# facontidavide/cloudini

Hardware: AMD Instinct MI355X
Metric: encode Mpoints/s (stage-1, pre-ZSTD) (higher is better)
Workload: dtype f32->i32 (u8 varint stream); 1 GPU; BASELINE configs[1]: 32 x 1000000-pt XYZI (f32 XYZ + u16 intensity, point_step 16) @1mm, stage-1 encode (pre-LZ4/ZSTD), V5 wire; clouds_per_gpu=32, points_per_cloud=1000000, point_step=16

## Files before the change

### cloudini_amd/csrc/stage1_finish.h

```cpp
#pragma once

namespace cldn {

constexpr uint32_t kFinMaxSegs = 96u + 2u * kMaxAdaptive;
constexpr uint32_t kFinItemUnits = 256u;
constexpr uint32_t kFinMaxItems = 512u;
constexpr uint32_t kFinSpinLimit = 1u << 22;

struct FinishArgs {
  const ChunkDesc* chunks;
  uint32_t n_chunks;
  uint32_t splits;
  const uint32_t* cloud_first_chunk;
  uint32_t n_clouds;
  const uint8_t* slots;
  uint64_t slot_stride;
  const Seg* segs;
  uint32_t segs_per_chunk;
  uint32_t subs;
  unsigned long long* rec;
  unsigned long long* rec2;
  unsigned long long* anchor;
  uint32_t epoch;
  uint32_t* ticket;
// ... 41 lines not shown

__device__ __forceinline__ void fin_layout(FinishLds& L, uint32_t n_segs, uint32_t skip0, uint32_t skip1,
                                           uint32_t dst_mis , uint32_t lane) {
  constexpr uint32_t K = (kFinMaxSegs + 63u) / 64u;
  uint32_t z[K], d[K], cnt[K], ibase[K];
  uint32_t payload = 0u;
#pragma unroll
  for (uint32_t k = 0; k < K; ++k) {
    const uint32_t s = lane + 64u * k;
    z[k] = s < n_segs ? L.seg[s].size : 0u;
    const uint32_t incl = wave_inclusive_scan(z[k]);
    d[k] = payload + incl - z[k];
    payload += (uint32_t)__builtin_amdgcn_readlane((int)incl, 63);
  }
  const uint32_t item_units = max(kFinItemUnits, (payload >> 4) / (kFinMaxItems - kFinMaxSegs - 8u) + 1u);
  uint32_t n_items = 0u;
#pragma unroll
  for (uint32_t k = 0; k < K; ++k) {
    const uint32_t s = lane + 64u * k;
    cnt[k] = 0u;
    if (z[k] != 0u && s != skip0 && s != skip1) {
      const uint32_t head = min(z[k], (16u - ((dst_mis + d[k]) & 15u)) & 15u);
      const uint32_t units = (z[k] - head) >> 4;
      cnt[k] = max(1u, (units + item_units - 1u) / item_units);
    }
    const uint32_t incl = wave_inclusive_scan(cnt[k]);
    ibase[k] = n_items + incl - cnt[k];
    n_items += (uint32_t)__builtin_amdgcn_readlane((int)incl, 63);
  }
#pragma unroll
  for (uint32_t k = 0; k < K; ++k) {
    const uint32_t s = lane + 64u * k;
    if (s < n_segs) L.doff[s] = d[k];
    for (uint32_t j = 0, it = ibase[k]; j < cnt[k] && it < kFinMaxItems; ++j, ++it) {
      L.item_seg[it] = s;
      L.item_u0[it] = j * item_units;
    }
  }
  if (lane == 0u) {
    L.n_items = min(n_items, kFinMaxItems);
    L.item_units = item_units;
    L.payload = payload;
  }
}

__device__ __forceinline__ void fin_copy(const FinishLds& L, const uint8_t* __restrict__ slot, uint8_t* __restrict__ chunk_out,
                                         uint32_t wid, uint32_t n_waves, uint32_t lane) {
  const uint32_t n_items = L.n_items, item_units = L.item_units;
  for (uint32_t it = wid; it < n_items; it += n_waves) {
    const uint32_t sidx = L.item_seg[it], u0 = L.item_u0[it];
    const Seg sg = L.seg[sidx];
    const uint8_t* src = slot + sg.off;
    uint8_t* dst = chunk_out + 4u + L.doff[sidx];
    const uint32_t size = sg.size;
    const uint32_t head = min(size, (uint32_t)((16u - (uint32_t)((uintptr_t)dst & 15u)) & 15u));
    const uint32_t body_units = (size - head) >> 4;
    const uint32_t tail = (size - head) & 15u;
    if (u0 == 0u) {
      if (lane < head) dst[lane] = src[lane];
      if (lane >= 32u && lane < 32u + tail) {
        const uint32_t k = head + body_units * 16u + (lane - 32u);
        dst[k] = src[k];
      }
    }
    const uint32_t sdw = head >> 2, sb = head & 3u;
    const uint4* src4 = reinterpret_cast<const uint4*>(src);
    uint4* dst4 = reinterpret_cast<uint4*>(dst + head);
    const uint32_t u1 = min(body_units, u0 + item_units);
    auto build = [&](const uint4& a, const uint4& b) __attribute__((always_inline)) {
      uint32_t w0, w1, w2, w3, w4;
      switch (sdw) {
        case 0: w0 = a.x; w1 = a.y; w2 = a.z; w3 = a.w; w4 = b.x; break;
        case 1: w0 = a.y; w1 = a.z; w2 = a.w; w3 = b.x; w4 = b.y; break;
        case 2: w0 = a.z; w1 = a.w; w2 = b.x; w3 = b.y; w4 = b.z; break;
        default: w0 = a.w; w1 = b.x; w2 = b.y; w3 = b.z; w4 = b.w; break;
      }
      uint4 o;
      o.x = funnel_bytes(w0, w1, sb);
      o.y = funnel_bytes(w1, w2, sb);
      o.z = funnel_bytes(w2, w3, sb);
      o.w = funnel_bytes(w3, w4, sb);
      return o;
    };
    if (u0 < u1) {
      const uint32_t last = head != 0u ? u1 : u1 - 1u;
      auto shl1 = [&](const uint4& a, const uint4& lane63) __attribute__((always_inline)) {
        uint4 r;
        r.x = (uint32_t)__builtin_amdgcn_update_dpp((int)lane63.x, (int)a.x, 0x130, 0xf, 0xf, false);
        r.y = (uint32_t)__builtin_amdgcn_update_dpp((int)lane63.y, (int)a.y, 0x130, 0xf, 0xf, false);
        r.z = (uint32_t)__builtin_amdgcn_update_dpp((int)lane63.z, (int)a.z, 0x130, 0xf, 0xf, false);
        r.w = (uint32_t)__builtin_amdgcn_update_dpp((int)lane63.w, (int)a.w, 0x130, 0xf, 0xf, false);
        return r;
      };
      auto lane0 = [&](const uint4& a) __attribute__((always_inline)) {
        return make_uint4((uint32_t)__builtin_amdgcn_readfirstlane((int)a.x), (uint32_t)__builtin_amdgcn_readfirstlane((int)a.y),
                          (uint32_t)__builtin_amdgcn_readfirstlane((int)a.z), (uint32_t)__builtin_amdgcn_readfirstlane((int)a.w));
      };
      auto ld = [&](uint32_t j, bool nt) __attribute__((always_inline)) {
        const uint4* q = src4 + min(j, last);
        if (!nt) return *q;
        typedef uint32_t u32x4 __attribute__((ext_vector_type(4)));
        const u32x4 v = __builtin_nontemporal_load(reinterpret_cast<const u32x4*>(q));
        return make_uint4(v.x, v.y, v.z, v.w);
      };
      auto st = [&](uint32_t j, const uint4& v, bool nt) __attribute__((always_inline)) {
        typedef uint32_t u32x4 __attribute__((ext_vector_type(4)));
        u32x4 q;
        q.x = v.x; q.y = v.y; q.z = v.z; q.w = v.w;
        if (nt) __builtin_nontemporal_store(q, reinterpret_cast<u32x4*>(dst4 + j));
        else dst4[j] = v;
      };
      auto rows_loop = [&](auto rows_tag, auto nt_tag) __attribute__((always_inline)) {
        constexpr uint32_t RW = decltype(rows_tag)::value;
        constexpr bool NT = decltype(nt_tag)::value;
        for (uint32_t jb = u0; jb < u1; jb += 64u * RW) {
          const uint32_t j = jb + lane;
          uint4 a[RW + 1];
#pragma unroll
          for (uint32_t r = 0; r < RW; ++r) a[r] = ld(j + 64u * r, NT);
          a[RW] = make_uint4(0u, 0u, 0u, 0u);
          if (lane == 63u && head != 0u) a[RW] = ld(j + 64u * (RW - 1u) + 1u, NT);
#pragma unroll
          for (uint32_t r = 0; r < RW; ++r) {
            const uint4 b = shl1(a[r], r + 1u < RW ? lane0(a[r + 1u]) : a[RW]);
            if (j + 64u * r < u1) st(j + 64u * r, build(a[r], b), NT);
          }
        }
      };
      rows_loop(std::integral_constant<uint32_t, 2>{}, std::true_type{});
    }
  }
}

__global__ __launch_bounds__(256) void k_chunk_sizes(const Seg* __restrict__ segs, uint32_t segs_per_chunk, uint32_t n_chunks,
                                                     uint32_t* __restrict__ chunk_payload, uint32_t* __restrict__ not_contiguous) {
  const uint32_t c = blockIdx.x * 256u + threadIdx.x;
  if (c >= n_chunks) return;
  uint32_t payload = 0u, next = 0xffffffffu;
  bool contiguous = true;
  for (uint32_t s = 0; s < segs_per_chunk; ++s) {
    const Seg sg = segs[(size_t)c * segs_per_chunk + s];
    if (sg.size == 0u) continue;
    if (next != 0xffffffffu && sg.off != next) contiguous = false;
    next = sg.off + sg.size;
    payload += sg.size;
  }
  chunk_payload[c] = payload;
  if (!contiguous) atomicOr(not_contiguous, 1u);
}

template <int T, int FUSE_BPV>
__global__ __launch_bounds__(T, (T == 1024 ? 4 : 8)) __attribute__((amdgpu_num_sgpr(80))) void k_finish(const FinishArgs A) {
  using RawT = typename std::conditional<FUSE_BPV == 4, uint32_t, uint16_t>::type;
  using P = Pal32<RawT>;
  __shared__ FinishLds L;
  extern __shared__ __attribute__((aligned(16))) uint8_t smem[];
  const uint32_t tid = threadIdx.x;
  const uint32_t lane = tid & 63u;
  const uint32_t wave = __builtin_amdgcn_readfirstlane(tid >> 6);

  if (A.test_timeout != 0u && A.use_ticket == 0u) {
    if (tid == 0u && blockIdx.x == 0u) atomicOr(A.status, (uint32_t)ST_FINISH_TIMEOUT);
    return;
  }
  if (tid == 0u) {
    L.ticket = A.use_ticket ? atomicAdd(A.ticket, 1u) : blockIdx.x;
    L.timeout = 0u;
    L.base = 0ull;
  }
  __syncthreads();
  const uint32_t t = L.ticket;
  const uint32_t c = t % A.n_chunks;
  const uint32_t y = t / A.n_chunks;
  const bool leader = (y == 0u);
  const ChunkDesc cd = A.chunks[c];
  const uint32_t n_segs = A.segs_per_chunk;
  if (tid < n_segs) L.seg[tid] = A.segs[(size_t)c * n_segs + tid];

  bool fuse = false, slow = false;
  uint32_t U = 0u;
  const uint32_t n = cd.n_points;
  const RawT* col = nullptr;
  uint16_t* first = nullptr;
  uint32_t s_a = 0xffffffffu, s_b = 0xffffffffu;
  if (FUSE_BPV != 0) {
    fuse = A.modes[cd.cloud * A.n_adaptive + A.fuse_field] == 1u;
    if (fuse) {
      s_a = A.subs + 2u * A.fuse_field;
      s_b = s_a + 1u;
      col = reinterpret_cast<const RawT*>(A.fuse_col) + cd.first_point;
      first = A.fuse_first + cd.first_point;
      if (leader) {
        const P p(smem);
        if (pal32_build<RawT, T>(p, col, n)) {
          U = p.misc[0];
        } else {
          slow = true;
          if (!pal32_slow_first<RawT, T>(p, col, n, first, A.status)) return;
          uint32_t mine = 0u;
          for (uint32_t i = tid; i < n; i += T) mine += first[i] == (uint16_t)i ? 1u : 0u;
          (void)block_exclusive_scan<T>(mine, p.wtot, &U);
          __syncthreads();
        }
        if (tid == 0u) fin_store(A.rec2 + c, ((unsigned long long)A.epoch << 32) | U);
      } else {
        if (tid == 0u) L.pad = fin_wait(A.rec2 + c, A.epoch, L);
        __syncthreads();
        if (L.timeout) {
          if (tid == 0u) atomicOr(A.status, (uint32_t)ST_FINISH_TIMEOUT);
          return;
        }
        U = L.pad;
      }
    }
  }
  __syncthreads();
  if (fuse && tid == 0u) {
    L.seg[s_a].size = 3u + U * (uint32_t)sizeof(RawT);
    L.seg[s_b].size = (palette_bits(U) * n + 7u) >> 3;
  }
  __syncthreads();

  if (tid == 0u) {
    uint32_t payload = 0u;
    for (uint32_t s = 0; s < n_segs; ++s) payload += L.seg[s].size;
    L.payload = payload;
    if (leader) fin_store(A.rec + c, ((unsigned long long)A.epoch << 32) | (payload + 4u));
  }
  {
    unsigned long long part = 0ull;
    const uint32_t blk = c >> 10;
    {
      constexpr uint32_t PER = 1024u / T;
      unsigned long long x[PER];
#pragma unroll
      for (uint32_t k = 0; k < PER; ++k) {
        const uint32_t j = (blk << 10) + tid + k * T;
        x[k] = j < c ? fin_load(A.rec + j) : ((unsigned long long)A.epoch << 32);
      }
      if (FUSE_BPV != 0 && fuse && leader && !slow) (void)pal32_rank<RawT, T>(P(smem), nullptr);
#pragma unroll
      for (uint32_t k = 0; k < PER; ++k) {
        const uint32_t j = (blk << 10) + tid + k * T;
        part += (uint32_t)(x[k] >> 32) == A.epoch ? (uint32_t)x[k] : fin_wait(A.rec + j, A.epoch, L);
      }
    }
    if (blk != 0u && tid == T - 1) {
      for (uint32_t spins = 0;; ++spins) {
        const unsigned long long x = fin_load(A.anchor + (blk - 1u));
        if (x != 0ull) {
          part += x - 1ull;
          break;
        }
        if (spins >= kFinSpinLimit || ((spins & 255u) == 255u && *(volatile uint32_t*)&L.timeout != 0u)) {
          L.timeout = 1u;
          break;
        }
        __builtin_amdgcn_s_sleep(2);
      }
    }
    uint32_t lo = (uint32_t)part, hi = (uint32_t)(part >> 32);
#pragma unroll
    for (int d = 32; d >= 1; d >>= 1) {
      const uint32_t olo = (uint32_t)__shfl_down((int)lo, d), ohi = (uint32_t)__shfl_down((int)hi, d);
      const unsigned long long sum = ((((unsigned long long)hi) << 32) | lo) + ((((unsigned long long)ohi) << 32) | olo);
      lo = (uint32_t)sum;
      hi = (uint32_t)(sum >> 32);
    }
    if (lane == 0u && (lo | hi)) atomicAdd(&L.base, (((unsigned long long)hi) << 32) | lo);
  }
  __syncthreads();
  if (L.timeout) {
    if (tid == 0u) atomicOr(A.status, (uint32_t)ST_FINISH_TIMEOUT);
    return;
  }
  const unsigned long long dst0 = L.base;
  if (wave == 0u) fin_layout(L, n_segs, s_a, s_b, (uint32_t)(((uintptr_t)A.out + dst0 + 4ull) & 15ull), lane);
  __syncthreads();
  const uint32_t payload = L.payload;
  if (dst0 + 4ull + payload > A.out_capacity) {
    if (tid == 0u && leader) atomicOr(A.status, (uint32_t)ST_OUT_OVERFLOW);
    return;
  }
  uint8_t* chunk_out = A.out + dst0;
  if (leader) {
    if (tid < 4u) chunk_out[tid] = (uint8_t)(payload >> (8u * tid));
    if (tid == 0u) {
      A.chunk_payload[c] = payload;
      A.chunk_dst[c] = dst0;
      if ((c & 1023u) == 1023u) fin_store(A.anchor + (c >> 10), dst0 + 4ull + payload + 1ull);
    }
    if (tid == 64u) {
      for (uint32_t k = cd.cloud + 1u; k-- > 0u && A.cloud_first_chunk[k] == c;) A.stream_offsets[k] = dst0;
      if (c + 1u == A.n_chunks)
        for (uint32_t k = A.n_clouds + 1u; k-- > 0u && A.cloud_first_chunk[k] == A.n_chunks;) A.stream_offsets[k] = dst0 + 4ull + payload;
    }
  }

  const uint8_t* slot = A.slots + (size_t)c * A.slot_stride;
  const bool leader_copies = !(fuse && A.splits >= 3u);
  const uint32_t wid = leader_copies ? y * (T / 64) + wave : (y - 1u) * (T / 64) + wave;
  const uint32_t n_waves = (leader_copies ? A.splits : A.splits - 1u) * (T / 64);
  const bool copies = leader_copies || !leader;
  const bool section_first = !fuse || !leader || (c & 1u) == 0u;
  if (!section_first && copies) fin_copy(L, slot, chunk_out, wid, n_waves, lane);
  if (FUSE_BPV != 0 && fuse && leader) {
    const P p(smem);
    uint8_t* sec = chunk_out + 4u + L.doff[s_a];
    uint8_t* idx = chunk_out + 4u + L.doff[s_b];
    if (!slow) {
      pal32_values<RawT, T>(p, sec + 3u);
      pal32_pack_chunk<RawT, T>(p, col, n, palette_bits(U), idx);
    } else {
      (void)pal32_slow_rank<RawT, T>(p, col, n, first, sec + 3u);
      pal32_slow_pack<RawT, T>(p, n, palette_bits(U), first, idx);
    }
    if (tid == 0u) {
      sec[0] = 1u;
      sec[1] = (uint8_t)(U & 0xffu);
      sec[2] = (uint8_t)((U >> 8) & 0xffu);
    }
  }
  if (section_first && copies) fin_copy(L, slot, chunk_out, wid, n_waves, lane);
}

}
```

### cloudini_amd/csrc/stage1_sections.h

```cpp
#pragma once

namespace cldn {

constexpr uint32_t kPalSeed = 2048u;

constexpr int kS2Threads = 1024;
constexpr uint32_t kS2PalSlots = 4096;
constexpr uint32_t kS2PalCapacity = 3072;
constexpr uint32_t kInf = 0xffffffffu;
constexpr uint32_t kProbeSlots = 8192;
constexpr uint32_t kProbeLds = kProbeSlots * 8u + 16u + 256u;

struct Pal2 {
  unsigned long long* keys;
  uint32_t* first;
  uint16_t* rank;
  uint32_t* misc;
  uint32_t* wtot;
};
constexpr uint32_t kS2PalLds = kS2PalSlots * 8u + (kS2PalSlots + 4u) * 4u + (kS2PalSlots + 8u) * 2u + 16u + 256u;

__device__ __forceinline__ Pal2 pal2_carve(uint8_t* lds) {
  Pal2 p;
  uint32_t o = 0;
// ... 167 lines not shown
    for (uint32_t w = threadIdx.x; w < 2048u; w += T) bm[w] = 0u;
    __syncthreads();
#pragma unroll
    for (uint32_t j = 0; j < VPT; ++j)
      if (j < cnt) atomicOr(&bm[(uint32_t)v[j] >> 5], 1u << ((uint32_t)v[j] & 31u));
    __syncthreads();
    uint32_t pc = 0u;
    for (uint32_t w = threadIdx.x; w < 2048u; w += T) pc += (uint32_t)__builtin_popcount(bm[w]);
    U = block_sum<T>(pc, wtot);
  } else {
    using Key = typename std::conditional<sizeof(RawT) == 8, unsigned long long, uint32_t>::type;
    constexpr Key kFreeKey = ~(Key)0;
    Key* keys = reinterpret_cast<Key*>(smem);
    uint32_t* cnt_l = wtot + 40;
    for (uint32_t sidx = threadIdx.x; sidx < slots; sidx += T) keys[sidx] = kFreeKey;
    if (threadIdx.x < 2u) cnt_l[threadIdx.x] = 0u;
    __syncthreads();
#pragma unroll
    for (uint32_t j = 0; j < VPT; ++j) {
      if (j < cnt) {
        const Key key = (Key)v[j];
        if (key == kFreeKey) {
          cnt_l[1] = 1u;
        } else {
          const uint32_t h32 = sizeof(RawT) == 8 ? hash_u64((uint64_t)key) * 0x9e3779b1u : (uint32_t)key * 0x9e3779b1u;
          uint32_t slot = (uint32_t)(((uint64_t)h32 * slots) >> 32);
          for (;;) {
            Key k = keys[slot];
            if (k == kFreeKey) {
              k = atomicCAS(&keys[slot], kFreeKey, key);
              if (k == kFreeKey) {
                atomicAdd(&cnt_l[0], 1u);
                break;
              }
            }
            if (k == key) break;
            slot = slot + 1u == slots ? 0u : slot + 1u;
          }
        }
      }
    }
    __syncthreads();
    U = cnt_l[0] + cnt_l[1];
    __syncthreads();
  }
  const uint32_t pal_size = 3u + U * (uint32_t)sizeof(RawT) + ((palette_bits(U) * n + 7u) >> 3);

  uint32_t mode = 0u, best = delta_size;
  if (pal_size < best) { best = pal_size; mode = 1u; }
  if (rle_size < best) { best = rle_size; mode = 2u; }
  if (drle_size < best) { mode = 3u; }
  return (uint8_t)mode;
}

template <typename RawT>
__device__ __forceinline__ uint8_t probe_mode(const RawT* col, uint32_t n, uint32_t type, uint8_t* smem) {
  uint32_t* wtot = reinterpret_cast<uint32_t*>(smem + kProbeSlots * 8u + 16u);
  return probe_mode_t<RawT, kS2Threads>([&](uint32_t i) { return col[i]; }, n, type, smem, kProbeSlots, wtot);
}

__global__ __launch_bounds__(kS2Threads) void k_probe_fast(const DevPlan plan, const ChunkDesc* __restrict__ chunks,
                                                           const uint32_t* __restrict__ cloud_first_chunk,
                                                           const ColumnPtrs cols, uint8_t* __restrict__ modes) {
  extern __shared__ __attribute__((aligned(16))) uint8_t smem[];
  const uint32_t cloud = blockIdx.x, a = blockIdx.y;
  uint8_t* mode_out = modes + cloud * plan.n_adaptive + a;
  const uint32_t fc = cloud_first_chunk[cloud];
  if (fc == cloud_first_chunk[cloud + 1u]) {
    if (threadIdx.x == 0) *mode_out = 0u;
    return;
  }
  const ChunkDesc cd = chunks[fc];
  const uint32_t n = cd.n_points > kProbePoints ? kProbePoints : cd.n_points;
  const uint32_t bpv = plan.adaptive[a].bpv, type = plan.adaptive[a].type;
  const uint8_t* col = cols.p[a] + (size_t)cd.first_point * bpv;
  uint8_t mode;
  if (bpv == 2u) mode = probe_mode<uint16_t>(reinterpret_cast<const uint16_t*>(col), n, type, smem);
  else if (bpv == 4u) mode = probe_mode<uint32_t>(reinterpret_cast<const uint32_t*>(col), n, type, smem);
  else mode = probe_mode<uint64_t>(reinterpret_cast<const uint64_t*>(col), n, type, smem);
  if (threadIdx.x == 0) *mode_out = mode;
}

template <typename RawT>
__global__ __launch_bounds__(kS2Threads) void k_section_palette(const DevPlan plan, const SectionFields fl,
                                                                const ChunkDesc* __restrict__ chunks,
                                                                const ColumnPtrs cols, const uint8_t* __restrict__ modes,
                                                                uint8_t* __restrict__ slots, uint64_t slot_stride,
                                                                uint64_t reg_stride, Seg* __restrict__ segs,
                                                                uint32_t segs_per_chunk, uint32_t subs,
                                                                uint8_t* __restrict__ handled_flags, uint32_t ) {
  constexpr int T = kS2Threads;
  constexpr int NW = T / 64;
  constexpr uint32_t ROUND = T * 8u;
  extern __shared__ __attribute__((aligned(16))) uint8_t smem[];
  const uint32_t c = blockIdx.x;
  const uint32_t a = fl.a[blockIdx.y];
  const ChunkDesc cd = chunks[c];
  if (modes[cd.cloud * plan.n_adaptive + a] != 1u) return;
  const uint32_t n = cd.n_points;
  const RawT* col = reinterpret_cast<const RawT*>(cols.p[a]) + cd.first_point;
  const uint32_t sec_off = (uint32_t)reg_stride + a * kSectionStride;
  uint8_t* dst = slots + (size_t)c * slot_stride + sec_off;
  const Pal2 p = pal2_carve(smem);
  const uint32_t tid = threadIdx.x;
  const uint32_t lane = tid & 63u;
  const uint32_t wave = __builtin_amdgcn_readfirstlane(tid >> 6);
  const uint32_t rounds = (n + ROUND - 1u) / ROUND;

  for (uint32_t s = tid; s < kS2PalSlots; s += T) p.keys[s] = ~0ull;
  for (uint32_t s = tid; s <= kS2PalSlots; s += T) p.first[s] = kInf;
  if (tid < 4u) p.misc[tid] = 0u;
  __syncthreads();

  for (uint32_t r = 0; r < rounds; ++r) {
    const uint32_t i0 = r * ROUND + tid * 8u;
    if (i0 < n) {
      RawT v[8];
      load8<RawT>(col, i0, n, v);
#pragma unroll
      for (int j = 0; j < 8; ++j) {
        if (i0 + (uint32_t)j < n) pal2_insert<RawT>(p, v[j], i0 + (uint32_t)j);
      }
    }
  }
  __syncthreads();
  if (p.misc[1] != 0u || p.misc[0] > kS2PalCapacity) return;

  uint32_t fmask = 0u;
  uint32_t incl[4], cnt[4];
#pragma unroll
  for (uint32_t r = 0; r < 4u; ++r) {
    uint32_t m = 0u;
    const uint32_t i0 = r * ROUND + tid * 8u;
    if (r < rounds && i0 < n) {
      RawT v[8];
      load8<RawT>(col, i0, n, v);
#pragma unroll
      for (int j = 0; j < 8; ++j) {
        if (i0 + (uint32_t)j < n && p.first[pal2_find<RawT>(p, v[j])] == i0 + (uint32_t)j) m |= 1u << j;
      }
    }
    fmask |= m << (8u * r);
    cnt[r] = (uint32_t)__builtin_popcount(m);
    incl[r] = wave_inclusive_scan(cnt[r]);
    if (lane == 63u) p.wtot[r * NW + wave] = incl[r];
  }
  __syncthreads();
  const uint32_t wincl = wave_inclusive_scan(p.wtot[lane]);
  const uint32_t U = (uint32_t)__builtin_amdgcn_readlane((int)wincl, 63);
#pragma unroll
  for (uint32_t r = 0; r < 4u; ++r) {
    const int f = (int)(r * NW + wave);
    const uint32_t rowbase = (f == 0) ? 0u : (uint32_t)__builtin_amdgcn_readlane((int)wincl, f - 1);
    const uint32_t m = (fmask >> (8u * r)) & 0xffu;
    if (m) {
      uint32_t rk = rowbase + incl[r] - cnt[r];
      const uint32_t i0 = r * ROUND + tid * 8u;
      RawT v[8];
      load8<RawT>(col, i0, n, v);
#pragma unroll
      for (int j = 0; j < 8; ++j) {
        if (m & (1u << j)) {
          p.rank[pal2_find<RawT>(p, v[j])] = (uint16_t)rk;
          const unsigned long long val = (unsigned long long)v[j];
          uint8_t* out = dst + 3u + (size_t)rk * sizeof(RawT);
#pragma unroll
          for (uint32_t k = 0; k < sizeof(RawT); ++k) out[k] = (uint8_t)(val >> (8u * k));
          ++rk;
        }
      }
    }
  }
  if (tid == 0) {
    dst[0] = 1u;
    dst[1] = (uint8_t)(U & 0xffu);
    dst[2] = (uint8_t)((U >> 8) & 0xffu);
  }
  __syncthreads();

  const uint32_t bits = palette_bits(U);
  if (bits != 0u && tid * 32u < n) {
    uint32_t* idx_out = reinterpret_cast<uint32_t*>(dst + kPaletteIndexOffset) + (size_t)tid * bits;
    uint64_t scratch = 0u;
    uint32_t held = 0u, w = 0u;
    for (uint32_t g = 0; g < 4u; ++g) {
      const uint32_t i0 = tid * 32u + g * 8u;
      if (i0 >= n) break;
      RawT v[8];
      load8<RawT>(col, i0, n, v);
#pragma unroll
      for (int j = 0; j < 8; ++j) {
        if (i0 + (uint32_t)j < n) {
          scratch |= ((uint64_t)p.rank[pal2_find<RawT>(p, v[j])]) << held;
          held += bits;
          if (held >= 32u) {
            idx_out[w++] = (uint32_t)scratch;
            scratch >>= 32;
            held -= 32u;
          }
        }
      }
    }
    if (held > 0u) idx_out[w] = (uint32_t)scratch;
  }
  if (tid == 0) {
    Seg s;
    s.off = sec_off;
    s.size = 3u + U * (uint32_t)sizeof(RawT);
    segs[(size_t)c * segs_per_chunk + subs + 2u * a] = s;
    s.off = sec_off + kPaletteIndexOffset;
    s.size = (bits * n + 7u) >> 3;
    segs[(size_t)c * segs_per_chunk + subs + 1u + 2u * a] = s;
    handled_flags[(size_t)c * plan.n_adaptive + a] = 1u;
  }
}

template <typename RawT>
struct Grp8 {
  uint32_t dw[2 * sizeof(RawT)];
  __device__ __forceinline__ uint32_t get(int j) const {
    return sizeof(RawT) == 2 ? ((dw[j >> 1] >> ((j & 1) * 16)) & 0xffffu) : dw[j];
  }
  __device__ __forceinline__ uint32_t get_dyn(uint32_t j) const {
    const uint32_t di = sizeof(RawT) == 2 ? (j >> 1) : j;
    uint32_t x = 0u;
#pragma unroll
    for (uint32_t k = 0; k < 2 * sizeof(RawT); ++k) {
      uint32_t a = dw[k];
      asm volatile("" : "+v"(a));
      x = di == k ? a : x;
    }
    return sizeof(RawT) == 2 ? ((x >> ((j & 1u) * 16u)) & 0xffffu) : x;
  }
};
template <typename RawT>
__device__ __forceinline__ Grp8<RawT> grp8_load(const RawT* col, uint32_t i0) {
  Grp8<RawT> g;
  __builtin_memcpy(g.dw, col + i0, 8u * sizeof(RawT));
  return g;
}

template <typename RawT>
struct Pal32 {
  using Word = typename std::conditional<sizeof(RawT) == 2, uint32_t, unsigned long long>::type;
  static constexpr uint32_t kShift = sizeof(RawT) == 2 ? 16u : 32u;
  static constexpr Word kFree = ~(Word)0;
  static constexpr uint32_t kLds = kS2PalSlots * (uint32_t)sizeof(Word) + 2u * kS2Threads * 4u + 16u + 256u;
  Word* tab;
  uint32_t* bitmap;
  uint32_t* prefix;
  uint32_t* misc;
  uint32_t* wtot;
  __device__ __forceinline__ explicit Pal32(uint8_t* lds) {
    uint32_t o = 0;
    tab = reinterpret_cast<Word*>(lds + o);
    o += kS2PalSlots * (uint32_t)sizeof(Word);
    bitmap = reinterpret_cast<uint32_t*>(lds + o);
    o += kS2Threads * 4u;
    prefix = reinterpret_cast<uint32_t*>(lds + o);
    o += kS2Threads * 4u;
    misc = reinterpret_cast<uint32_t*>(lds + o);
    o += 16u;
    wtot = reinterpret_cast<uint32_t*>(lds + o);
  }
  static __device__ __forceinline__ uint32_t home(uint32_t v) { return (v * 0x9e3779b1u) >> 20; }
  static __device__ __forceinline__ uint32_t key_of(Word w) { return (uint32_t)(w >> kShift); }
  static __device__ __forceinline__ uint32_t low_of(Word w) { return (uint32_t)w & 0xffffu; }

  __device__ __forceinline__ void insert(uint32_t v, uint32_t index, Word w) const {
    const Word mine = ((Word)v << kShift) | index;
    uint32_t slot = home(v);
    uint32_t probes = 0u;
    for (;;) {
      if (misc[0] > kS2PalCapacity) return;
      if (w == kFree) {
        w = atomicCAS(&tab[slot], kFree, mine);
        if (w == kFree) {
          atomicAdd(&misc[0], 1u);
          return;
        }
      }
      if (key_of(w) == v) {
        if (low_of(w) > index) atomicMin(&tab[slot], mine);
        return;
      }
      slot = (slot + 1u) & (kS2PalSlots - 1u);
      if (++probes > kS2PalSlots) {
        misc[1] = 1u;
        return;
      }
      w = tab[slot];
    }
  }
  __device__ __forceinline__ uint32_t find_rank(uint32_t v, Word w) const {
    uint32_t slot = home(v);
    while (w == kFree || key_of(w) != v) {
      slot = (slot + 1u) & (kS2PalSlots - 1u);
      w = tab[slot];
    }
    return low_of(w);
  }
};

template <typename RawT, uint32_t BITS, bool AHEAD = false>
__device__ __forceinline__ void pal32_pack(const Pal32<RawT>& p, const RawT* col, uint32_t i0, uint32_t n, uint32_t cnt,
                                           uint8_t* out) {
  using P = Pal32<RawT>;
  uint32_t w[BITS];
#pragma unroll
  for (uint32_t k = 0; k < BITS; ++k) w[k] = 0u;
  Grp8<RawT> grp[AHEAD ? 4 : 1];
  if constexpr (AHEAD) {
#pragma unroll
    for (int g = 0; g < 4; ++g) grp[g] = grp8_load<RawT>(col, i0 + 8u * g < n ? i0 + 8u * g : i0);
  }
#pragma unroll
  for (int g = 0; g < 4; ++g) {
    uint32_t v[8];
    if constexpr (AHEAD) {
#pragma unroll
      for (int j = 0; j < 8; ++j) v[j] = grp[g].get(j);
    } else {
      RawT rv[8];
#pragma unroll
      for (int j = 0; j < 8; ++j) rv[j] = (RawT)0;
      if (i0 + 8u * g < n) load8<RawT>(col, i0 + 8u * g, n, rv);
#pragma unroll
      for (int j = 0; j < 8; ++j) v[j] = (uint32_t)rv[j];
    }
    typename P::Word tw[8];
#pragma unroll
    for (int j = 0; j < 8; ++j) tw[j] = p.tab[P::home(v[j])];
#pragma unroll
    for (int j = 0; j < 8; ++j) {
      const uint32_t e = (uint32_t)(8 * g + j);
      uint32_t x = 0u;
      if (e < cnt) {
        const bool hit = tw[j] != P::kFree && P::key_of(tw[j]) == v[j];
        x = hit ? P::low_of(tw[j]) : p.find_rank(v[j], tw[j]);
      }
      const uint32_t bit = e * BITS;
      w[bit >> 5] |= x << (bit & 31u);
      if ((bit & 31u) + BITS > 32u) w[(bit >> 5) + 1u] |= x >> (32u - (bit & 31u));
    }
  }
  const uint32_t n_bytes = (cnt * BITS + 7u) >> 3;
  const uint32_t n_dw = n_bytes >> 2;
  if (n_dw == BITS && BITS % 4u == 0u) {
#pragma unroll
    for (uint32_t k = 0; k < BITS; k += 4u) {
      const uint4 q = make_uint4(w[k], w[k + 1u], w[k + 2u], w[k + 3u]);
      __builtin_memcpy(out + 4u * k, &q, 16);
    }
  } else {
#pragma unroll
    for (uint32_t k = 0; k < BITS; ++k) {
      if (k < n_dw) __builtin_memcpy(out + 4u * k, &w[k], 4);
      else if (k == n_dw) {
        for (uint32_t b = 0; b < (n_bytes & 3u); ++b) out[4u * k + b] = (uint8_t)(w[k] >> (8u * b));
      }
    }
  }
}


template <typename RawT, int T>
__device__ __forceinline__ bool pal32_build(const Pal32<RawT>& p, const RawT* col, uint32_t n) {
  using P = Pal32<RawT>;
  using Word = typename P::Word;
  constexpr uint32_t WPT = kS2Threads / T;
  const uint32_t tid = threadIdx.x;
  uint32_t seedv[kPalSeed / T];
#pragma unroll
  for (uint32_t r = 0; r < kPalSeed / T; ++r) seedv[r] = (uint32_t)col[min(r * T + tid, n - 1u)];
  for (uint32_t s = tid; s < kS2PalSlots; s += T) p.tab[s] = P::kFree;
#pragma unroll
  for (uint32_t w = 0; w < WPT; ++w) p.bitmap[w * T + tid] = 0u;
  if (tid < 4u) p.misc[tid] = 0u;
  __syncthreads();
#pragma unroll
  for (uint32_t r = 0; r < kPalSeed / T; ++r) {
    const uint32_t i = r * T + tid;
    if (i < n) p.insert(seedv[r], i, p.tab[P::home(seedv[r])]);
  }
  __syncthreads();
  constexpr uint32_t STEPS = 4096u / T;
  constexpr uint32_t GB = sizeof(RawT) == 2 ? (STEPS < 8u ? STEPS : 8u) : 4u;
#pragma unroll
  for (uint32_t b = 0; b < STEPS; b += GB) {
    Grp8<RawT> g[GB];
#pragma unroll
    for (uint32_t k = 0; k < GB; ++k) {
      const uint32_t i0 = ((b + k) * T + tid) * 8u;
      g[k] = grp8_load<RawT>(col, i0 < n ? i0 : 0u);
    }
#pragma unroll
    for (uint32_t k = 0; k < GB; ++k) {
      const uint32_t i0 = ((b + k) * T + tid) * 8u;
      if (i0 >= n || i0 + 8u <= kPalSeed) continue;
      Word w[8];
#pragma unroll
      for (int j = 0; j < 8; ++j) w[j] = p.tab[P::home(g[k].get(j))];
      uint32_t todo = 0u;
#pragma unroll
      for (int j = 0; j < 8; ++j) {
        const uint32_t idx = i0 + (uint32_t)j;
        const bool settled = w[j] != P::kFree && P::key_of(w[j]) == g[k].get(j) && P::low_of(w[j]) <= idx;
        todo |= (idx < n && !settled) ? (1u << j) : 0u;
      }
      while (todo != 0u) {
        const uint32_t j = (uint32_t)__builtin_ctz(todo);
        todo &= todo - 1u;
        const uint32_t v = g[k].get_dyn(j);
        p.insert(v, i0 + j, p.tab[P::home(v)]);
      }
    }
  }
  __syncthreads();
  return p.misc[1] == 0u && p.misc[0] <= kS2PalCapacity;
}

template <typename RawT, int T>
__device__ __forceinline__ uint32_t pal32_rank(const Pal32<RawT>& p, uint8_t* vals_out) {
  using P = Pal32<RawT>;
  using Word = typename P::Word;
  constexpr uint32_t WPT = kS2Threads / T;
  const uint32_t tid = threadIdx.x;
#pragma unroll
  for (uint32_t q = 0; q < kS2PalSlots / T; ++q) {
    const Word w = p.tab[q * T + tid];
    if (w != P::kFree) atomicOr(&p.bitmap[P::low_of(w) >> 5], 1u << (P::low_of(w) & 31u));
  }
  __syncthreads();
  uint32_t U;
  {
    uint32_t pc[WPT], mine = 0u;
#pragma unroll
    for (uint32_t w = 0; w < WPT; ++w) {
      pc[w] = (uint32_t)__builtin_popcount(p.bitmap[WPT * tid + w]);
      mine += pc[w];
    }
    uint32_t run = block_exclusive_scan<T>(mine, p.wtot, &U);
#pragma unroll
    for (uint32_t w = 0; w < WPT; ++w) {
      p.prefix[WPT * tid + w] = run;
      run += pc[w];
    }
  }
  __syncthreads();
#pragma unroll
  for (uint32_t q = 0; q < kS2PalSlots / T; ++q) {
    const Word w = p.tab[q * T + tid];
    if (w != P::kFree) {
      const uint32_t f = P::low_of(w);
      const uint32_t rk = p.prefix[f >> 5] + (uint32_t)__builtin_popcount(p.bitmap[f >> 5] & ((1u << (f & 31u)) - 1u));
      p.tab[q * T + tid] = (w & ~(Word)0xffffu) | rk;
      if (vals_out != nullptr) {
        const uint32_t val = P::key_of(w);
        uint8_t* out = vals_out + (size_t)rk * sizeof(RawT);
#pragma unroll
        for (uint32_t b = 0; b < sizeof(RawT); ++b) out[b] = (uint8_t)(val >> (8u * b));
      }
    }
  }
  __syncthreads();
  return U;
}

template <typename RawT, int T>
__device__ __forceinline__ void pal32_values(const Pal32<RawT>& p, uint8_t* vals_out) {
  using P = Pal32<RawT>;
  using Word = typename P::Word;
  const uint32_t tid = threadIdx.x;
#pragma unroll
  for (uint32_t q = 0; q < kS2PalSlots / T; ++q) {
    const Word w = p.tab[q * T + tid];
    if (w != P::kFree) {
      const uint32_t val = P::key_of(w);
      uint8_t* out = vals_out + (size_t)P::low_of(w) * sizeof(RawT);
#pragma unroll
      for (uint32_t b = 0; b < sizeof(RawT); ++b) out[b] = (uint8_t)(val >> (8u * b));
    }
  }
}

template <typename RawT, int T>
__device__ __forceinline__ void pal32_pack_chunk(const Pal32<RawT>& p, const RawT* col, uint32_t n, uint32_t bits,
                                                 uint8_t* idx_out) {
  constexpr uint32_t WPT = kS2Threads / T;
  const uint32_t tid = threadIdx.x;
  for (uint32_t g = 0; g < WPT; ++g) {
    const uint32_t grp = g * T + tid;
    const uint32_t i0 = grp * 32u;
    const uint32_t cnt = i0 < n ? min(32u, n - i0) : 0u;
    if (bits != 0u && cnt != 0u) {
      uint8_t* o = idx_out + (size_t)grp * bits * 4u;
      switch (bits) {
        case 1: pal32_pack<RawT, 1, T == 1024>(p, col, i0, n, cnt, o); break;
        case 2: pal32_pack<RawT, 2, T == 1024>(p, col, i0, n, cnt, o); break;
        case 3: pal32_pack<RawT, 3, T == 1024>(p, col, i0, n, cnt, o); break;
        case 4: pal32_pack<RawT, 4, T == 1024>(p, col, i0, n, cnt, o); break;
        case 5: pal32_pack<RawT, 5, T == 1024>(p, col, i0, n, cnt, o); break;
        case 6: pal32_pack<RawT, 6, T == 1024>(p, col, i0, n, cnt, o); break;
        case 7: pal32_pack<RawT, 7, T == 1024>(p, col, i0, n, cnt, o); break;
        case 8: pal32_pack<RawT, 8, T == 1024>(p, col, i0, n, cnt, o); break;
        case 9: pal32_pack<RawT, 9, T == 1024>(p, col, i0, n, cnt, o); break;
        case 10: pal32_pack<RawT, 10, T == 1024>(p, col, i0, n, cnt, o); break;
        case 11: pal32_pack<RawT, 11, T == 1024>(p, col, i0, n, cnt, o); break;
        default: pal32_pack<RawT, 12, T == 1024>(p, col, i0, n, cnt, o); break;
      }
    }
  }
}

constexpr uint32_t kPalSlowMaxParts = 4096;

template <typename RawT>
__device__ __forceinline__ uint32_t pal32_part(uint32_t v, uint32_t parts) {
  if (sizeof(RawT) == 2) return (v * parts) >> 16;
  uint32_t h = v * 0x85ebca6bu;
  h ^= h >> 15;
  h *= 0xc2b2ae35u;
  return (uint32_t)(((uint64_t)h * parts) >> 32);
}

template <typename RawT, int T>
__device__ __forceinline__ bool pal32_slow_first(const Pal32<RawT> p, const RawT* col, uint32_t n, uint16_t* first, uint32_t* status) {
  using P = Pal32<RawT>;
  const uint32_t tid = threadIdx.x;
  uint32_t parts = 32u;
  for (;;) {
    bool ok = true;
    for (uint32_t part = 0; part < parts && ok; ++part) {
      __syncthreads();
      for (uint32_t s = tid; s < kS2PalSlots; s += T) p.tab[s] = P::kFree;
      if (tid < 4u) p.misc[tid] = 0u;
      __syncthreads();
      for (uint32_t i = tid; i < n; i += T) {
        const uint32_t v = (uint32_t)col[i];
        if (pal32_part<RawT>(v, parts) == part) p.insert(v, i, p.tab[P::home(v)]);
      }
      __syncthreads();
      ok = p.misc[1] == 0u && p.misc[0] <= kS2PalCapacity;
      if (!ok) break;
      for (uint32_t i = tid; i < n; i += T) {
        const uint32_t v = (uint32_t)col[i];
        if (pal32_part<RawT>(v, parts) == part) {
          uint32_t slot = P::home(v);
          typename P::Word w = p.tab[slot];
          while (w == P::kFree || P::key_of(w) != v) {
            slot = (slot + 1u) & (kS2PalSlots - 1u);
            w = p.tab[slot];
          }
          first[i] = (uint16_t)P::low_of(w);
        }
      }
    }
    if (ok) break;
    if (sizeof(RawT) == 2 || parts >= kPalSlowMaxParts) {
      if (tid == 0) atomicOr(status, (uint32_t)ST_PALETTE_FULL);
      return false;
    }
    parts *= 4u;
  }
  __threadfence_block();
  __syncthreads();
  return true;
}

template <typename RawT, int T>
__device__ __forceinline__ uint32_t pal32_slow_rank(const Pal32<RawT> p, const RawT* col, uint32_t n, const uint16_t* first,
                                    uint8_t* vals_out) {
  constexpr uint32_t WPT = kS2Threads / T;
  const uint32_t tid = threadIdx.x;
  uint32_t U;
  uint32_t pc[WPT], bm[WPT], mine = 0u;
#pragma unroll
  for (uint32_t w = 0; w < WPT; ++w) {
    const uint32_t word = WPT * tid + w;
    uint32_t m = 0u;
    for (uint32_t b = 0; b < 32u; ++b) {
      const uint32_t i = word * 32u + b;
      if (i < n && first[i] == (uint16_t)i) m |= 1u << b;
    }
    bm[w] = m;
    p.bitmap[word] = m;
    pc[w] = (uint32_t)__builtin_popcount(m);
    mine += pc[w];
  }
  uint32_t run = block_exclusive_scan<T>(mine, p.wtot, &U);
#pragma unroll
  for (uint32_t w = 0; w < WPT; ++w) {
    const uint32_t word = WPT * tid + w;
    p.prefix[word] = run;
    uint32_t m = bm[w];
    uint32_t rk = run;
    while (m) {
      const uint32_t b = (uint32_t)__builtin_ctz(m);
      m &= m - 1u;
      const uint64_t val = (uint64_t)col[word * 32u + b];
      uint8_t* out = vals_out + (size_t)rk * sizeof(RawT);
#pragma unroll
      for (uint32_t k = 0; k < sizeof(RawT); ++k) out[k] = (uint8_t)(val >> (8u * k));
      ++rk;
    }
    run += pc[w];
  }
  __syncthreads();
  return U;
}

template <typename RawT, int T>
__device__ __forceinline__ void pal32_slow_pack(const Pal32<RawT> p, uint32_t n, uint32_t bits, const uint16_t* first, uint8_t* idx_out) {
  constexpr uint32_t WPT = kS2Threads / T;
  const uint32_t tid = threadIdx.x;
  if (bits == 0u) return;
  for (uint32_t g = 0; g < WPT; ++g) {
    const uint32_t grp = g * T + tid;
    const uint32_t i0 = grp * 32u;
    if (i0 >= n) continue;
    const uint32_t cnt = min(32u, n - i0);
    uint8_t* o = idx_out + (size_t)grp * bits * 4u;
    uint64_t scratch = 0u;
    uint32_t held = 0u, w = 0u;
    for (uint32_t j = 0; j < cnt; ++j) {
      const uint32_t f = first[i0 + j];
      const uint32_t rk = p.prefix[f >> 5] + (uint32_t)__builtin_popcount(p.bitmap[f >> 5] & ((1u << (f & 31u)) - 1u));
      scratch |= ((uint64_t)rk) << held;
      held += bits;
      if (held >= 32u) {
        const uint32_t d = (uint32_t)scratch;
        __builtin_memcpy(o + 4u * w, &d, 4);
        ++w;
        scratch >>= 32;
        held -= 32u;
      }
    }
    for (uint32_t b = 0; b < ((held + 7u) >> 3); ++b) o[4u * w + b] = (uint8_t)(scratch >> (8u * b));
  }
}

template <typename RawT, int T = kS2Threads>
__global__ __launch_bounds__(T, (T == 512 ? 8 : 4)) __attribute__((amdgpu_num_sgpr(80))) void k_section_palette32(
    const DevPlan plan, const SectionFields fl, const ChunkDesc* __restrict__ chunks, const ColumnPtrs cols,
    const uint8_t* __restrict__ modes, uint8_t* __restrict__ slots, uint64_t slot_stride, uint64_t reg_stride,
    Seg* __restrict__ segs, uint32_t segs_per_chunk, uint32_t subs, uint8_t* __restrict__ handled_flags, uint32_t append,
    const ColumnPtrs first_cols, uint32_t* __restrict__ status) {
  static_assert(sizeof(RawT) == 2 || sizeof(RawT) == 4, "16- or 32-bit keys");
  static_assert(kS2Threads * 32u == 32768u && (T == kS2Threads || 2 * T == kS2Threads), "bitmap words per thread: 1 or 2");
  using P = Pal32<RawT>;
  extern __shared__ __attribute__((aligned(16))) uint8_t smem[];
  const uint32_t c = blockIdx.x;
  const uint32_t a = fl.a[blockIdx.y];
  const ChunkDesc cd = chunks[c];
  if (modes[cd.cloud * plan.n_adaptive + a] != 1u) return;
  const uint32_t n = cd.n_points;
  const RawT* col = reinterpret_cast<const RawT*>(cols.p[a]) + cd.first_point;
  const uint32_t sec_off = append ? segs[(size_t)c * segs_per_chunk].size : (uint32_t)reg_stride + a * kSectionStride;
  uint8_t* dst = slots + (size_t)c * slot_stride + sec_off;
  const P p(smem);
  const uint32_t tid = threadIdx.x;

  uint32_t U;
  if (pal32_build<RawT, T>(p, col, n)) {
    U = p.misc[0];
    (void)pal32_rank<RawT, T>(p, dst + 3u);
    pal32_pack_chunk<RawT, T>(p, col, n, palette_bits(U), dst + 3u + U * (uint32_t)sizeof(RawT));
  } else {
    uint16_t* first = reinterpret_cast<uint16_t*>(first_cols.p[a]) + cd.first_point;
    if (!pal32_slow_first<RawT, T>(p, col, n, first, status)) return;
    uint32_t mine = 0u;
    for (uint32_t i = tid; i < n; i += T) mine += first[i] == (uint16_t)i ? 1u : 0u;
    (void)block_exclusive_scan<T>(mine, p.wtot, &U);
    __syncthreads();
    (void)pal32_slow_rank<RawT, T>(p, col, n, first, dst + 3u);
    pal32_slow_pack<RawT, T>(p, n, palette_bits(U), first, dst + 3u + U * (uint32_t)sizeof(RawT));
  }
  if (tid == 0) {
    dst[0] = 1u;
    dst[1] = (uint8_t)(U & 0xffu);
    dst[2] = (uint8_t)((U >> 8) & 0xffu);
    Seg s;
    s.off = sec_off;
    s.size = 3u + U * (uint32_t)sizeof(RawT) + ((palette_bits(U) * n + 7u) >> 3);
    segs[(size_t)c * segs_per_chunk + subs + 2u * a] = s;
    s.size = 0u;
    segs[(size_t)c * segs_per_chunk + subs + 1u + 2u * a] = s;
    handled_flags[(size_t)c * plan.n_adaptive + a] = 1u;
  }
}

constexpr uint32_t kD32Ring = 65536;
constexpr uint32_t kD32Lds = kD32Ring + 256u;

template <typename RawT>
__device__ __forceinline__ void section_delta32_body(const DevPlan& plan, uint32_t c, uint32_t a, const ChunkDesc& cd, const ColumnPtrs& cols,
                                                     uint8_t* __restrict__ slots, uint64_t slot_stride, uint64_t reg_stride,
                                                     Seg* __restrict__ segs, uint32_t segs_per_chunk, uint32_t subs,
                                                     uint8_t* __restrict__ handled_flags, uint32_t append, uint8_t* smem) {
  static_assert(sizeof(RawT) == 2 || sizeof(RawT) == 4, "differences of at most 33 bits");
  constexpr int T = kS2Threads;
  uint32_t* ring = reinterpret_cast<uint32_t*>(smem);
  uint32_t* wtot = reinterpret_cast<uint32_t*>(smem + kD32Ring);
  const uint32_t n = cd.n_points;
  const uint32_t type = plan.adaptive[a].type;
  const RawT* col = reinterpret_cast<const RawT*>(cols.p[a]) + cd.first_point;
  const uint32_t sec_off = append ? segs[(size_t)c * segs_per_chunk].size : (uint32_t)reg_stride + a * kSectionStride;
  uint8_t* dst = slots + (size_t)c * slot_stride + sec_off;
  const uint32_t tid = threadIdx.x;
  Grp8<RawT> pre[4];
  RawT pre_prev[4];
#pragma unroll
  for (uint32_t q = 0; q < 4u; ++q) {
    const uint32_t i0 = q * (T * 8u) + threadIdx.x * 8u;
    pre[q] = grp8_load<RawT>(col, i0 < n ? i0 : 0u);
    pre_prev[q] = col[(i0 > 0u && i0 < n) ? i0 - 1u : 0u];
  }
  for (uint32_t i = tid; i < kD32Ring / 16u; i += T) reinterpret_cast<uint4*>(ring)[i] = make_uint4(0u, 0u, 0u, 0u);
  __syncthreads();

  uint32_t R = 1u, F = 0u;
#pragma unroll
  for (uint32_t q = 0; q < 4u; ++q) {
    const uint32_t i0 = q * (T * 8u) + tid * 8u;
    if (q * (T * 8u) >= n) break;
    RawT v[8];
#pragma unroll
    for (int j = 0; j < 8; ++j) v[j] = (RawT)pre[q].get(j);
    int64_t prev = (i0 > 0u && i0 < n) ? int_field_as_i64((uint64_t)pre_prev[q], type) : 0;
    uint32_t w0[8], w1[8], lens = 0u, total = 0u;
#pragma unroll
    for (int j = 0; j < 8; ++j) {
      const int64_t cur = int_field_as_i64((uint64_t)v[j], type);
      const int64_t d = (int64_t)((uint64_t)cur - (uint64_t)prev);
      prev = cur;
      const uint64_t u = (((uint64_t)d << 1) ^ (uint64_t)(d >> 63)) + 1ull;
      const uint32_t bl = (u >> 32) ? (64u - (uint32_t)__builtin_clzll(u)) : (32u - (uint32_t)__builtin_clz((uint32_t)u));
      const uint32_t l = (i0 + (uint32_t)j < n) ? groups7(bl) : 0u;
      w0[j] = spread28((uint32_t)u & 0x0fffffffu) | cont_mask(l ? l - 1u : 0u);
      w1[j] = (uint32_t)(u >> 28);
      lens |= l << (4 * j);
      total += l;
    }
    uint32_t tile_total;
    uint32_t off = R + block_exclusive_scan<T>(total, wtot, &tile_total);
#pragma unroll
    for (int j = 0; j < 8; ++j) {
      const uint32_t l = (lens >> (4 * j)) & 0xfu;
      if (l) ring_put5<kD32Ring, false>(ring, off, w0[j], w1[j], l, 0u);
      off += l;
    }
    const uint32_t r_end = R + tile_total;
    const bool last = (q + 1u) * (T * 8u) >= n;
    const uint32_t target = last ? ((r_end + 15u) & ~15u) : (r_end & ~15u);
    __syncthreads();
    ring_flush_n<T, kD32Ring>(ring, dst, F, target);
    F = target;
    R = r_end;
    __syncthreads();
  }
  if (tid == 0) {
    Seg sg;
    sg.off = sec_off;
    sg.size = R;
    segs[(size_t)c * segs_per_chunk + subs + 2u * a] = sg;
    sg.off = sec_off;
    sg.size = 0u;
    segs[(size_t)c * segs_per_chunk + subs + 1u + 2u * a] = sg;
    handled_flags[(size_t)c * plan.n_adaptive + a] = 1u;
  }
}

template <typename RawT>
__device__ __forceinline__ void section_runs_body(const DevPlan& plan, uint32_t c, uint32_t a, const ChunkDesc& cd, uint32_t mode,
                                                  const ColumnPtrs& cols, uint8_t* __restrict__ slots, uint64_t slot_stride,
                                                  uint64_t reg_stride, Seg* __restrict__ segs, uint32_t segs_per_chunk, uint32_t subs,
                                                  uint8_t* __restrict__ handled_flags, uint32_t append, uint8_t* smem) {
  static_assert(sizeof(RawT) == 2 || sizeof(RawT) == 4, "differences of at most 33 bits");
  constexpr int T = kS2Threads;
  uint32_t* wtot = reinterpret_cast<uint32_t*>(smem);
  const bool delta = (mode == 3u);
  const uint32_t n = cd.n_points;
  const uint32_t type = plan.adaptive[a].type;
  const RawT* col = reinterpret_cast<const RawT*>(cols.p[a]) + cd.first_point;
  const uint32_t sec_off = append ? segs[(size_t)c * segs_per_chunk].size : (uint32_t)reg_stride + a * kSectionStride;
  uint8_t* dst = slots + (size_t)c * slot_stride + sec_off;
  const uint32_t tid = threadIdx.x;
  const uint32_t i0 = tid * 32u;
  const uint32_t cnt = i0 < n ? min(32u, n - i0) : 0u;
  auto as64 = [&](RawT r) { return int_field_as_i64((uint64_t)r, type); };

  uint64_t key[32];
  uint64_t key_before = 0u;
  {
    RawT v[32];
    Grp8<RawT> g8[4];
#pragma unroll
    for (uint32_t g = 0; g < 4u; ++g) g8[g] = grp8_load<RawT>(col, i0 + 8u * g < n ? i0 + 8u * g : 0u);
    const RawT pm1r = col[(cnt && i0 >= 1u) ? i0 - 1u : 0u];
    const RawT pm2r = col[(cnt && i0 >= 2u) ? i0 - 2u : 0u];
#pragma unroll
    for (int g = 0; g < 4; ++g)
#pragma unroll
      for (int j = 0; j < 8; ++j) v[8 * g + j] = (i0 + (uint32_t)(8 * g + j) < n) ? (RawT)g8[g].get(j) : (RawT)0;
    const RawT pm1 = (cnt && i0 >= 1u) ? pm1r : (RawT)0;
    const RawT pm2 = (cnt && i0 >= 2u) ? pm2r : (RawT)0;
    if (delta) {
      int64_t prev = i0 >= 1u ? as64(pm1) : 0;
      key_before = (uint64_t)prev - (uint64_t)(i0 >= 2u ? as64(pm2) : 0);
#pragma unroll
      for (int j = 0; j < 32; ++j) {
        const int64_t cur = as64(v[j]);
        key[j] = (uint64_t)cur - (uint64_t)prev;
        prev = cur;
// ... 89 lines not shown
```

Baseline: 133,800 Mpoints/s.

## Repack palette indices per 8-value group with batched loads and deferred misses

The palette index packer now gives each thread one 8-value group per step instead of 32 values, so consecutive threads write adjacent small outputs. Loads for several groups are issued up front, separated from the compute by a scheduling barrier. Hash-table misses are collected into a bitmask and resolved afterwards, and base pointers are forced uniform with readfirstlane. The copy ordering in the finish step is also simplified to always run after palette emission. This trades more loop iterations and some register pressure for better coalescing and latency hiding.

```diff
diff --git a/cloudini_amd/csrc/stage1_finish.h b/cloudini_amd/csrc/stage1_finish.h
--- a/cloudini_amd/csrc/stage1_finish.h
+++ b/cloudini_amd/csrc/stage1_finish.h
@@ -367,8 +367,6 @@
   const uint32_t wid = leader_copies ? y * (T / 64) + wave : (y - 1u) * (T / 64) + wave;
   const uint32_t n_waves = (leader_copies ? A.splits : A.splits - 1u) * (T / 64);
   const bool copies = leader_copies || !leader;
-  const bool section_first = !fuse || !leader || (c & 1u) == 0u;
-  if (!section_first && copies) fin_copy(L, slot, chunk_out, wid, n_waves, lane);
   if (FUSE_BPV != 0 && fuse && leader) {
     const P p(smem);
     uint8_t* sec = chunk_out + 4u + L.doff[s_a];
@@ -386,7 +384,7 @@
       sec[2] = (uint8_t)((U >> 8) & 0xffu);
     }
   }
-  if (section_first && copies) fin_copy(L, slot, chunk_out, wid, n_waves, lane);
-}
-
-}
+  if (copies) fin_copy(L, slot, chunk_out, wid, n_waves, lane);
+}
+
+}
diff --git a/cloudini_amd/csrc/stage1_sections.h b/cloudini_amd/csrc/stage1_sections.h
--- a/cloudini_amd/csrc/stage1_sections.h
+++ b/cloudini_amd/csrc/stage1_sections.h
@@ -493,64 +493,55 @@
   }
 };
 
-template <typename RawT, uint32_t BITS, bool AHEAD = false>
-__device__ __forceinline__ void pal32_pack(const Pal32<RawT>& p, const RawT* col, uint32_t i0, uint32_t n, uint32_t cnt,
-                                           uint8_t* out) {
+template <typename RawT, uint32_t BITS>
+__device__ __forceinline__ void pal32_pack(const Pal32<RawT>& p, const Grp8<RawT>& g, uint32_t cnt, uint8_t* out) {
   using P = Pal32<RawT>;
-  uint32_t w[BITS];
-#pragma unroll
-  for (uint32_t k = 0; k < BITS; ++k) w[k] = 0u;
-  Grp8<RawT> grp[AHEAD ? 4 : 1];
-  if constexpr (AHEAD) {
-#pragma unroll
-    for (int g = 0; g < 4; ++g) grp[g] = grp8_load<RawT>(col, i0 + 8u * g < n ? i0 + 8u * g : i0);
-  }
-#pragma unroll
-  for (int g = 0; g < 4; ++g) {
-    uint32_t v[8];
-    if constexpr (AHEAD) {
-#pragma unroll
-      for (int j = 0; j < 8; ++j) v[j] = grp[g].get(j);
+  constexpr uint32_t NW = (BITS + 3u) / 4u;
+  typename P::Word tw[8];
+#pragma unroll
+  for (int j = 0; j < 8; ++j) tw[j] = p.tab[P::home(g.get(j))];
+  uint32_t x[8], todo = 0u;
+#pragma unroll
+  for (int j = 0; j < 8; ++j) {
+    const bool hit = tw[j] != P::kFree && P::key_of(tw[j]) == g.get(j);
+    x[j] = (uint32_t)j < cnt ? P::low_of(tw[j]) : 0u;
+    todo |= ((uint32_t)j < cnt && !hit) ? (1u << j) : 0u;
+  }
+  while (todo != 0u) {
+    const uint32_t j = (uint32_t)__builtin_ctz(todo);
+    todo &= todo - 1u;
+    const uint32_t v = g.get_dyn(j);
+    const uint32_t r = p.find_rank(v, p.tab[P::home(v)]);
+#pragma unroll
+    for (uint32_t k = 0; k < 8u; ++k) x[k] = j == k ? r : x[k];
+  }
+  uint32_t w[NW];
+#pragma unroll
+  for (uint32_t k = 0; k < NW; ++k) w[k] = 0u;
+#pragma unroll
+  for (uint32_t j = 0; j < 8u; ++j) {
+    const uint32_t bit = j * BITS;
+    w[bit >> 5] |= x[j] << (bit & 31u);
+    if ((bit & 31u) + BITS > 32u) w[(bit >> 5) + 1u] |= x[j] >> (32u - (bit & 31u));
+  }
+  if (cnt == 8u) {
+    constexpr uint32_t ND = BITS / 4u;
+    if (ND != 0u) __builtin_memcpy(out, w, 4u * ND);
+    if (ND != 0u && (BITS & 3u) == 3u) {
+      const uint32_t e = (w[ND - 1u] >> 24) | (w[NW - 1u] << 8);
+      __builtin_memcpy(out + BITS - 4u, &e, 4);
     } else {
-      RawT rv[8];
-#pragma unroll
-      for (int j = 0; j < 8; ++j) rv[j] = (RawT)0;
-      if (i0 + 8u * g < n) load8<RawT>(col, i0 + 8u * g, n, rv);
-#pragma unroll
-      for (int j = 0; j < 8; ++j) v[j] = (uint32_t)rv[j];
-    }
-    typename P::Word tw[8];
-#pragma unroll
-    for (int j = 0; j < 8; ++j) tw[j] = p.tab[P::home(v[j])];
-#pragma unroll
-    for (int j = 0; j < 8; ++j) {
-      const uint32_t e = (uint32_t)(8 * g + j);
-      uint32_t x = 0u;
-      if (e < cnt) {
-        const bool hit = tw[j] != P::kFree && P::key_of(tw[j]) == v[j];
-        x = hit ? P::low_of(tw[j]) : p.find_rank(v[j], tw[j]);
-      }
-      const uint32_t bit = e * BITS;
-      w[bit >> 5] |= x << (bit & 31u);
-      if ((bit & 31u) + BITS > 32u) w[(bit >> 5) + 1u] |= x >> (32u - (bit & 31u));
-    }
-  }
-  const uint32_t n_bytes = (cnt * BITS + 7u) >> 3;
-  const uint32_t n_dw = n_bytes >> 2;
-  if (n_dw == BITS && BITS % 4u == 0u) {
-#pragma unroll
-    for (uint32_t k = 0; k < BITS; k += 4u) {
-      const uint4 q = make_uint4(w[k], w[k + 1u], w[k + 2u], w[k + 3u]);
-      __builtin_memcpy(out + 4u * k, &q, 16);
-    }
-  } else {
-#pragma unroll
-    for (uint32_t k = 0; k < BITS; ++k) {
-      if (k < n_dw) __builtin_memcpy(out + 4u * k, &w[k], 4);
-      else if (k == n_dw) {
-        for (uint32_t b = 0; b < (n_bytes & 3u); ++b) out[4u * k + b] = (uint8_t)(w[k] >> (8u * b));
-      }
-    }
+      if (BITS & 2u) {
+        const uint16_t h = (uint16_t)w[NW - 1u];
+        __builtin_memcpy(out + 4u * ND, &h, 2);
+      }
+      if (BITS & 1u) out[BITS - 1u] = (uint8_t)(w[NW - 1u] >> ((BITS & 2u) * 8u));
+    }
+  } else if (cnt != 0u) {
+    const uint32_t n_bytes = (cnt * BITS + 7u) >> 3;
+#pragma unroll
+    for (uint32_t k = 0; k < NW; ++k)
+      for (uint32_t b = 0; b < 4u && 4u * k + b < n_bytes; ++b) out[4u * k + b] = (uint8_t)(w[k] >> (8u * b));
   }
 }
 
@@ -675,32 +666,57 @@
   }
 }
 
+template <typename RawT, int T, uint32_t BITS>
+__device__ __forceinline__ void pal32_pack_rounds(const Pal32<RawT>& p, const RawT* col, uint32_t n, uint8_t* idx_out) {
+  constexpr uint32_t STEPS = 4096u / T;
+  constexpr uint32_t GB = sizeof(RawT) == 2 ? (STEPS < 8u ? STEPS : 8u) : 4u;
+  uint32_t tid = threadIdx.x;
+  asm volatile("" : "+v"(tid));
+#pragma unroll
+  for (uint32_t b = 0; b < STEPS; b += GB) {
+    Grp8<RawT> g[GB];
+#pragma unroll
+    for (uint32_t k = 0; k < GB; ++k) {
+      const uint32_t i0 = ((b + k) * T + tid) * 8u;
+      g[k] = grp8_load<RawT>(col, i0 < n ? i0 : 0u);
+    }
+    __builtin_amdgcn_sched_barrier(0);
+#pragma unroll
+    for (uint32_t k = 0; k < GB; ++k) {
+      const uint32_t grp = (b + k) * T + tid;
+      const uint32_t i0 = grp * 8u;
+      pal32_pack<RawT, BITS>(p, g[k], i0 < n ? min(8u, n - i0) : 0u, idx_out + (size_t)grp * BITS);
+    }
+  }
+}
+
+template <typename X>
+__device__ __forceinline__ X* uniform_ptr(X* q) {
+  const uintptr_t a = (uintptr_t)q;
+  const uint32_t lo = (uint32_t)__builtin_amdgcn_readfirstlane((int)(uint32_t)a);
+  const uint32_t hi = (uint32_t)__builtin_amdgcn_readfirstlane((int)(uint32_t)(a >> 32));
+  return (X*)(((uintptr_t)hi << 32) | lo);
+}
+
 template <typename RawT, int T>
 __device__ __forceinline__ void pal32_pack_chunk(const Pal32<RawT>& p, const RawT* col, uint32_t n, uint32_t bits,
                                                  uint8_t* idx_out) {
-  constexpr uint32_t WPT = kS2Threads / T;
-  const uint32_t tid = threadIdx.x;
-  for (uint32_t g = 0; g < WPT; ++g) {
-    const uint32_t grp = g * T + tid;
-    const uint32_t i0 = grp * 32u;
-    const uint32_t cnt = i0 < n ? min(32u, n - i0) : 0u;
-    if (bits != 0u && cnt != 0u) {
-      uint8_t* o = idx_out + (size_t)grp * bits * 4u;
-      switch (bits) {
-        case 1: pal32_pack<RawT, 1, T == 1024>(p, col, i0, n, cnt, o); break;
-        case 2: pal32_pack<RawT, 2, T == 1024>(p, col, i0, n, cnt, o); break;
-        case 3: pal32_pack<RawT, 3, T == 1024>(p, col, i0, n, cnt, o); break;
-        case 4: pal32_pack<RawT, 4, T == 1024>(p, col, i0, n, cnt, o); break;
-        case 5: pal32_pack<RawT, 5, T == 1024>(p, col, i0, n, cnt, o); break;
-        case 6: pal32_pack<RawT, 6, T == 1024>(p, col, i0, n, cnt, o); break;
-        case 7: pal32_pack<RawT, 7, T == 1024>(p, col, i0, n, cnt, o); break;
-        case 8: pal32_pack<RawT, 8, T == 1024>(p, col, i0, n, cnt, o); break;
-        case 9: pal32_pack<RawT, 9, T == 1024>(p, col, i0, n, cnt, o); break;
-        case 10: pal32_pack<RawT, 10, T == 1024>(p, col, i0, n, cnt, o); break;
-        case 11: pal32_pack<RawT, 11, T == 1024>(p, col, i0, n, cnt, o); break;
-        default: pal32_pack<RawT, 12, T == 1024>(p, col, i0, n, cnt, o); break;
-      }
-    }
+  col = uniform_ptr(col);
+  idx_out = uniform_ptr(idx_out);
+  switch (bits) {
+    case 0: break;
+    case 1: pal32_pack_rounds<RawT, T, 1>(p, col, n, idx_out); break;
+    case 2: pal32_pack_rounds<RawT, T, 2>(p, col, n, idx_out); break;
+    case 3: pal32_pack_rounds<RawT, T, 3>(p, col, n, idx_out); break;
+    case 4: pal32_pack_rounds<RawT, T, 4>(p, col, n, idx_out); break;
+    case 5: pal32_pack_rounds<RawT, T, 5>(p, col, n, idx_out); break;
+    case 6: pal32_pack_rounds<RawT, T, 6>(p, col, n, idx_out); break;
+    case 7: pal32_pack_rounds<RawT, T, 7>(p, col, n, idx_out); break;
+    case 8: pal32_pack_rounds<RawT, T, 8>(p, col, n, idx_out); break;
+    case 9: pal32_pack_rounds<RawT, T, 9>(p, col, n, idx_out); break;
+    case 10: pal32_pack_rounds<RawT, T, 10>(p, col, n, idx_out); break;
+    case 11: pal32_pack_rounds<RawT, T, 11>(p, col, n, idx_out); break;
+    default: pal32_pack_rounds<RawT, T, 12>(p, col, n, idx_out); break;
   }
 }
 
```

After: 142,500 Mpoints/s (median of 6 runs). +6.5%, better.
